# 17LiQi/MultimodalSignal

Hardware: AMD Instinct MI355X
Metric: train windows/sec (higher is better)
Workload: dtype f32; 1 GPU; CnnGruAttentionModel full train step (fwd+CE+bwd+Adam, dropout 0.5, BN batch stats), B=8192 windows/GPU x (6 ch, 3840 samples = 60 s @ 64 Hz), random-init weights; BASELINE.json configs[4] shape, the per-step work of configs[1]; batch_per_gpu=8192, channels=6, samples=3840, classes=2, parallelism=replica x1

## Files before the change

multimodalsignal_amd/csrc/frontend.hip:

```cpp
#include "msig_dev.h"

template <int CT, bool EO_ONLY = false>
__global__ __launch_bounds__(256) void gate_kernel(const float* __restrict__ x, const float* __restrict__ W1,
                                                   const float* __restrict__ W2, float* __restrict__ mean_out,
                                                   float* __restrict__ pre_out, float* __restrict__ s_out,
                                                   float* __restrict__ eo_out, int C, int T, int Cr, const FoldCtx fc) {
  FOLD_BEGIN; FS(x); FS(W1); FS(W2); FS(mean_out); FS(pre_out); FS(s_out); FS(eo_out);
  __shared__ float red[4][MSIG_MAX_C];
  __shared__ float red_eo[4][2 * MSIG_MAX_C];
  __shared__ float mean_s[MSIG_MAX_C];
  __shared__ float hid_s[MSIG_MAX_C / 4];
  const int b = blockIdx.x, tid = threadIdx.x, lane = tid & 63, w = tid >> 6;
  const float* xb = x + (size_t)b * C * T;
  if (CT > 0 && (T & 3) == 0) {
    constexpr int CN = CT > 0 ? CT : 1;
    float acc[CN], ev[CN], od[CN];
#pragma unroll
    for (int c = 0; c < CN; ++c) acc[c] = ev[c] = od[c] = 0.f;
    const int T4 = T / 4;
    constexpr int U = CN <= 4 ? 4 : 2;
    for (int i0 = tid; i0 < T4; i0 += 256 * U) {
      float4 q[U][CN];
#pragma unroll
      for (int u = 0; u < U; ++u) {
        const int i = i0 + 256 * u < T4 ? i0 + 256 * u : i0;
#pragma unroll
        for (int c = 0; c < CN; ++c) q[u][c] = ((const float4*)xb)[(size_t)c * T4 + i];
      }
#pragma unroll
      for (int u = 0; u < U; ++u)
        if (i0 + 256 * u < T4) {
#pragma unroll
          for (int c = 0; c < CN; ++c) {
            if (!EO_ONLY) acc[c] += (q[u][c].x + q[u][c].y) + (q[u][c].z + q[u][c].w);
            ev[c] += q[u][c].x + q[u][c].z; od[c] += q[u][c].y + q[u][c].w;
          }
        }
    }
#pragma unroll
    for (int c = 0; c < CN; ++c) {
      if (!EO_ONLY) {
        const float a = wave_sum(acc[c]);
        if (lane == 0) red[w][c] = a;
      }
      if (eo_out) {
        const float e = wave_sum(ev[c]), o = wave_sum(od[c]);
        if (lane == 0) { red_eo[w][2 * c] = e; red_eo[w][2 * c + 1] = o; }
      }
    }
  } else
  for (int c = 0; c < C; ++c) {
    const float* xc = xb + (size_t)c * T;
    float acc = 0.f, ev = 0.f, od = 0.f;
// ... 502 lines not shown
  __shared__ float red[256 * 8];
  const int c4 = threadIdx.x % C4;
  float s1[4] = {0.f, 0.f, 0.f, 0.f}, s2[4] = {0.f, 0.f, 0.f, 0.f};
  float mean[4], invstd[4];
#pragma unroll
  for (int e = 0; e < 4; ++e) { mean[e] = stat[c4 * 4 + e]; invstd[e] = stat[CH + c4 * 4 + e]; }
  const int64_t total = (int64_t)B * L * C4;
  for (int64_t i = (int64_t)blockIdx.x * 256 + threadIdx.x; i < total; i += (int64_t)gridDim.x * 256) {
    const int64_t bt = i / C4;
    const int t = (int)(bt % L), b = (int)(bt / L);
    RoutedRaw r = routed_load<CH>(dp_a, code, b, t, P, c4);
    if (dp_b) {
      const RoutedRaw r2 = routed_load<CH>(dp_b, code, b, t, P, c4);
      r.g0.x += r2.g0.x; r.g0.y += r2.g0.y; r.g0.z += r2.g0.z; r.g0.w += r2.g0.w;
      r.g1.x += r2.g1.x; r.g1.y += r2.g1.y; r.g1.z += r2.g1.z; r.g1.w += r2.g1.w;
    }
    const float4 d = routed_dz(r, t, P);
    const float4 yq = *(const float4*)(y + ((size_t)b * L + t) * CH + c4 * 4);
    *(float4*)(dz + ((size_t)b * L + t) * CH + c4 * 4) = d;
    const float dv[4] = {d.x, d.y, d.z, d.w}, yv[4] = {yq.x, yq.y, yq.z, yq.w};
#pragma unroll
    for (int e = 0; e < 4; ++e) { s1[e] += dv[e]; s2[e] += dv[e] * (yv[e] - mean[e]) * invstd[e]; }
  }
#pragma unroll
  for (int e = 0; e < 4; ++e) { red[threadIdx.x * 8 + e] = s1[e]; red[threadIdx.x * 8 + 4 + e] = s2[e]; }
  __syncthreads();
  if (threadIdx.x < 2 * CH) {
    const int which = threadIdx.x / CH, ch = threadIdx.x % CH, cc4 = ch / 4, e = ch % 4;
    float acc = 0.f;
    for (int t = cc4; t < 256; t += C4) acc += red[t * 8 + which * 4 + e];
    part[(size_t)blockIdx.x * 2 * CH + threadIdx.x] = acc;
  }
}

__global__ __launch_bounds__(FIN_THREADS) void bn_bwd_finalize_kernel(const float* __restrict__ part, int nrows, int CH, double count,
                                                              float* __restrict__ cstat, float* __restrict__ dgamma,
                                                              float* __restrict__ dbeta, int batch_stats, const FoldCtx fc) {
  FOLD_BEGIN; FS(part); FS(cstat); FS(dgamma); FS(dbeta);
  __shared__ double red[FIN_THREADS];
  const int tid = threadIdx.x, ncol = 2 * CH;
  fin_colsums(part, nrows, ncol, red);
  if (tid < ncol) {
    const double s = red[tid];
    if (tid < CH) dbeta[tid] = (float)s; else dgamma[tid - CH] = (float)s;
    cstat[tid] = batch_stats ? (float)(s / count) : 0.f;
  }
}

#define D2_UCH 128
#define D2_ROWS (D2_UCH + 2)
#define D2_PS 36
#define W2_PROWS (2 * D2_UCH + 3)

__global__ __launch_bounds__(256) void conv2_bwd_kernel(const float* __restrict__ dz2, const float* __restrict__ y2,
                                                        const float* __restrict__ stat, const float* __restrict__ cstat,
                                                        const float* __restrict__ w2, const float* __restrict__ p1,
                                                        float* __restrict__ dp1, float* __restrict__ part, int B, int P1, int L2,
                                                        const FoldCtx fc) {
  FOLD_BEGIN; FS(dz2); FS(y2); FS(stat); FS(cstat); FS(w2); FS(p1); FS(dp1); FS(part);
  __shared__ __attribute__((aligned(16))) float ds_[D2_ROWS * D2_PS];
  __shared__ __attribute__((aligned(16))) float ps[W2_PROWS * C2_PS];
  const int tid = threadIdx.x, lane = tid & 63, w = tid >> 6, li = lane & 15, lq = lane >> 4;
  float Ae[24], Ao[16];
#pragma unroll
  for (int m = 0; m < 24; ++m) Ae[m] = w2[((lq * 8 + (m & 7)) * 16 + li) * 5 + 2 * (m >> 3)];
#pragma unroll
  for (int m = 0; m < 16; ++m) Ao[m] = w2[((lq * 8 + (m & 7)) * 16 + li) * 5 + 1 + 2 * (m >> 3)];
  f32x4 acc[2][5];
#pragma unroll
  for (int ob = 0; ob < 2; ++ob)
#pragma unroll
    for (int kk = 0; kk < 5; ++kk) acc[ob][kk] = (f32x4){0.f, 0.f, 0.f, 0.f};
  const int nchunk = (L2 + D2_UCH - 1) / D2_UCH;
  const int nitems = B * nchunk;
  float bn_mean[4], bn_inv[4], bn_sc[4], bn_c1[4], bn_c2[4];
#pragma unroll
  for (int e = 0; e < 4; ++e) {
    const int ch = (tid & 7) * 4 + e;
    bn_mean[e] = stat[ch]; bn_inv[e] = stat[32 + ch]; bn_sc[e] = stat[64 + ch]; bn_c1[e] = cstat[ch]; bn_c2[e] = cstat[32 + ch];
  }
  constexpr int ND4 = (D2_ROWS * 8 + 255) / 256, NP4 = (W2_PROWS * 4 + 255) / 256;
  float4 dr[ND4], yr[ND4], qr[NP4];
  auto prefetch = [&](int item) {
    const int b = item / nchunk, t0 = (item - b * nchunk) * D2_UCH, base = 2 * t0 - 2;
#pragma unroll
    for (int j = 0; j < ND4; ++j) {
      const int i = tid + 256 * j, row = i >> 3, c4 = i & 7, t = t0 - 1 + row;
      const int tc = t < 0 ? 0 : (t > L2 - 1 ? L2 - 1 : t);
      dr[j] = *(const float4*)(dz2 + ((size_t)b * L2 + tc) * 32 + c4 * 4);
      yr[j] = *(const float4*)(y2 + ((size_t)b * L2 + tc) * 32 + c4 * 4);
    }
#pragma unroll
    for (int j = 0; j < NP4; ++j) {
      const int i = tid + 256 * j, row = i >> 2, c4 = i & 3, src = base + row;
      const int sc = src < 0 ? 0 : (src > P1 - 1 ? P1 - 1 : src);
      qr[j] = *(const float4*)(p1 + ((size_t)b * P1 + sc) * 16 + c4 * 4);
    }
  };
  if ((int)blockIdx.x < nitems) prefetch(blockIdx.x);
  for (int item = blockIdx.x; item < nitems; item += gridDim.x) {
    const int b = item / nchunk, t0 = (item - b * nchunk) * D2_UCH;
    __syncthreads();
#pragma unroll
    for (int j = 0; j < ND4; ++j) {
      const int i = tid + 256 * j, row = i >> 3, c4 = i & 7, t = t0 - 1 + row;
      if (i < D2_ROWS * 8) {
        const float4 dzv = dr[j];
        float4 q;
        q.x = bn_sc[0] * (dzv.x - bn_c1[0] - (yr[j].x - bn_mean[0]) * bn_inv[0] * bn_c2[0]);
        q.y = bn_sc[1] * (dzv.y - bn_c1[1] - (yr[j].y - bn_mean[1]) * bn_inv[1] * bn_c2[1]);
        q.z = bn_sc[2] * (dzv.z - bn_c1[2] - (yr[j].z - bn_mean[2]) * bn_inv[2] * bn_c2[2]);
        q.w = bn_sc[3] * (dzv.w - bn_c1[3] - (yr[j].w - bn_mean[3]) * bn_inv[3] * bn_c2[3]);
        if (t < 0 || t >= L2) q = make_float4(0.f, 0.f, 0.f, 0.f);
        *(float4*)&ds_[row * D2_PS + c4 * 4] = q;
      }
    }
    const int base = 2 * t0 - 2;
#pragma unroll
    for (int j = 0; j < NP4; ++j) {
      const int i = tid + 256 * j, row = i >> 2, c4 = i & 3, src = base + row;
      if (i < W2_PROWS * 4) {
        float4 q = qr[j];
        if (src < 0 || src >= P1) q = make_float4(0.f, 0.f, 0.f, 0.f);
        *(float4*)&ps[row * C2_PS + c4 * 4] = q;
      }
    }
    __syncthreads();
    if (item + (int)gridDim.x < nitems) prefetch(item + gridDim.x);
#pragma unroll
    for (int ubi = 0; ubi < 2; ++ubi) {
      const int ul = (w * 2 + ubi) * 16 + li;
      f32x4 ae0 = {0.f, 0.f, 0.f, 0.f}, ae1 = {0.f, 0.f, 0.f, 0.f}, ao0 = {0.f, 0.f, 0.f, 0.f}, ao1 = {0.f, 0.f, 0.f, 0.f};
#pragma unroll
      for (int ti = 0; ti < 3; ++ti) {
        const float* rowp = &ds_[(ul + 2 - ti) * D2_PS + lq * 8];
        const float4 q0 = *(const float4*)rowp, q1 = *(const float4*)(rowp + 4);
        const float qv[8] = {q0.x, q0.y, q0.z, q0.w, q1.x, q1.y, q1.z, q1.w};
#pragma unroll
        for (int mm = 0; mm < 8; ++mm) {
          if (mm & 1) ae1 = mfma16(Ae[ti * 8 + mm], qv[mm], ae1); else ae0 = mfma16(Ae[ti * 8 + mm], qv[mm], ae0);
          if (ti < 2) { if (mm & 1) ao1 = mfma16(Ao[ti * 8 + mm], qv[mm], ao1); else ao0 = mfma16(Ao[ti * 8 + mm], qv[mm], ao0); }
        }
      }
      const int u = t0 + ul;
      if (2 * u < P1)
        *(float4*)(dp1 + ((size_t)b * P1 + 2 * u) * 16 + lq * 4) = make_float4(ae0[0] + ae1[0], ae0[1] + ae1[1], ae0[2] + ae1[2], ae0[3] + ae1[3]);
      if (2 * u + 1 < P1)
        *(float4*)(dp1 + ((size_t)b * P1 + 2 * u + 1) * 16 + lq * 4) = make_float4(ao0[0] + ao1[0], ao0[1] + ao1[1], ao0[2] + ao1[2], ao0[3] + ao1[3]);
    }
#pragma unroll 2
    for (int m = 0; m < D2_UCH / 16; ++m) {
      const int tl = w * 32 + 4 * m + lq;
      const float a0 = ds_[(tl + 1) * D2_PS + li], a1 = ds_[(tl + 1) * D2_PS + 16 + li];
#pragma unroll
      for (int kk = 0; kk < 5; ++kk) {
        const float bv = ps[(2 * tl + kk) * C2_PS + li];
        acc[0][kk] = mfma16(a0, bv, acc[0][kk]);
        acc[1][kk] = mfma16(a1, bv, acc[1][kk]);
      }
    }
  }
  __syncthreads();
  float* red = ds_;
  for (int ww = 0; ww < 4; ++ww) {
    if (w == ww) {
#pragma unroll
      for (int ob = 0; ob < 2; ++ob)
#pragma unroll
        for (int kk = 0; kk < 5; ++kk)
#pragma unroll
          for (int e = 0; e < 4; ++e) {
            const int o = ob * 16 + lq * 4 + e, c = li;
            const int idx = (o * 16 + c) * 5 + kk;
            red[idx] = (ww == 0 ? 0.f : red[idx]) + acc[ob][kk][e];
          }
    }
    __syncthreads();
  }
  for (int i = tid; i < 2560; i += 256) part[(size_t)blockIdx.x * 2560 + i] = red[i];
}

struct QuadRaw { float4 g[3], y[4]; unsigned c[3]; };
__device__ __forceinline__ void quad_load(QuadRaw& r, const float* __restrict__ dp1, const uint8_t* __restrict__ code1,
                                          const float* __restrict__ y1, int b, int tq, int L1, int P1, int sc4) {
  const int tqc = tq < L1 - 4 ? tq : L1 - 4;
  const int ph = tqc >> 1, ph2 = ph + 2 < P1 ? ph + 2 : P1 - 1;
  const float* dpb = dp1 + (size_t)b * P1 * 16;
  const uint8_t* cb = code1 + (size_t)b * P1 * 4;
  const float* yb = y1 + (size_t)b * L1 * 16;
  const unsigned o = (unsigned)(ph * 16 + sc4 * 4), oc = (unsigned)(ph * 4 + sc4), oy = (unsigned)(tqc * 16 + sc4 * 4);
  r.g[0] = *(const float4*)(dpb + o); r.g[1] = *(const float4*)(dpb + o + 16); r.g[2] = *(const float4*)(dpb + (unsigned)(ph2 * 16 + sc4 * 4));
  r.c[0] = cb[oc]; r.c[1] = cb[oc + 4]; r.c[2] = cb[(unsigned)(ph2 * 4 + sc4)];
#pragma unroll
  for (int j = 0; j < 4; ++j) r.y[j] = *(const float4*)(yb + oy + 16 * j);
}
__device__ __forceinline__ void quad_dz_xhat(const QuadRaw& r, int tq, int L1, int P1, const float* bn_mean, const float* bn_inv,
                                             float4 dz[4], float4 xh[4]) {
  const bool inside = tq < L1, has2 = (tq >> 1) + 2 < P1;
  const float g0[4] = {r.g[0].x, r.g[0].y, r.g[0].z, r.g[0].w}, g1[4] = {r.g[1].x, r.g[1].y, r.g[1].z, r.g[1].w},
              g2[4] = {r.g[2].x, r.g[2].y, r.g[2].z, r.g[2].w};
  float d[4][4];
#pragma unroll
  for (int e = 0; e < 4; ++e) {
    const unsigned c0 = (r.c[0] >> (2 * e)) & 3u, c1 = (r.c[1] >> (2 * e)) & 3u, c2 = has2 ? (r.c[2] >> (2 * e)) & 3u : 3u;
    d[0][e] = c0 == 1u ? g0[e] : 0.f;
    d[1][e] = (c0 == 2u ? g0[e] : 0.f) + (c1 == 0u ? g1[e] : 0.f);
    d[2][e] = c1 == 1u ? g1[e] : 0.f;
    d[3][e] = (c1 == 2u ? g1[e] : 0.f) + (c2 == 0u ? g2[e] : 0.f);
  }
#pragma unroll
  for (int j = 0; j < 4; ++j) {
    float4 dq = make_float4(d[j][0], d[j][1], d[j][2], d[j][3]), h;
    h.x = (r.y[j].x - bn_mean[0]) * bn_inv[0];
    h.y = (r.y[j].y - bn_mean[1]) * bn_inv[1];
    h.z = (r.y[j].z - bn_mean[2]) * bn_inv[2];
    h.w = (r.y[j].w - bn_mean[3]) * bn_inv[3];
    if (!inside) { dq = make_float4(0.f, 0.f, 0.f, 0.f); h = dq; }
    dz[j] = dq; xh[j] = h;
  }
}

#define G1_TCH 256
#ifndef CONV1_BWD_PIPE
#define CONV1_BWD_PIPE 1
#endif
#define CONV1_BWD_WGS (CONV1_BWD_PIPE ? 2 : 4)
#define G1_MAXNB 7
#define G1_XS (C1_XW + 4)
#define G1_QS 80
__device__ __forceinline__ int g1_row(int r) { return (r >> 2) * G1_QS + (r & 3) * 16; }

__host__ __device__ inline int conv1_bwd_cps(int B, int nchunk) { return B >= 256 ? nchunk : (nchunk + 7) / 8; }
// ... 89 lines not shown
          h.y = (yv.y - bn_mean[1]) * bn_inv[1];
          h.z = (yv.z - bn_mean[2]) * bn_inv[2];
          h.w = (yv.w - bn_mean[3]) * bn_inv[3];
          if (t >= L1) { dq = make_float4(0.f, 0.f, 0.f, 0.f); h = dq; }
          *(float4*)&dzs[g1_row(row) + c4 * 4] = dq;
          *(float4*)&xhs[g1_row(row) + c4 * 4] = h;
        }
      }
      __syncthreads();
      if (pipe) {
        if (ch + 1 < ch_hi) prefetch(b, ch + 1);
        else if (item + (int)gridDim.x < nitems) { const int ni = item + gridDim.x; prefetch(ni / SEG, (ni % SEG) * CPS); }
      }
#pragma unroll
      for (int m = 0; m < G1_TCH / 16; ++m) {
        const float a1 = dzs[aoff + G1_QS * m], a2 = xhs[aoff + G1_QS * m];
        s1 += a1; s2 = fmaf(a1, a2, s2);
#pragma unroll
        for (int nb = 0; nb < NBC; ++nb)
          if (CT > 0 || nb < NB) {
            const float bv = xs[coff[nb] + 8 * m];
            acc1[nb] = mfma16(a1, bv, acc1[nb]);
            acc2[nb] = mfma16(a2, bv, acc2[nb]);
          }
      }
    }
    __syncthreads();
#pragma unroll
    for (int nb = 0; nb < NBC; ++nb)
      if (CT > 0 || nb < NB) {
#pragma unroll
        for (int e = 0; e < 4; ++e) {
          red[((w * 2 + 0) * 16 + lq * 4 + e) * NB16 + nb * 16 + li] = acc1[nb][e];
          red[((w * 2 + 1) * 16 + lq * 4 + e) * NB16 + nb * 16 + li] = acc2[nb][e];
        }
      }
    __syncthreads();
    {
      float* gw = g1w + (size_t)item * 32 * NB16;
      for (int i = tid; i < 32 * NB16; i += 256)
        gw[i] = (red[i] + red[32 * NB16 + i]) + (red[64 * NB16 + i] + red[96 * NB16 + i]);
    }
  }
  __syncthreads();
  red[(w * 4 + lq) * 32 + li] = s1;
  red[(w * 4 + lq) * 32 + 16 + li] = s2;
  __syncthreads();
  if (tid < 32) {
    float a = 0.f;
    for (int q = 0; q < 16; ++q) a += red[q * 32 + tid];
    bpart[(size_t)blockIdx.x * 32 + tid] = a;
  }
}

template <bool GATED = true>
__global__ __launch_bounds__(256) void conv1_bwd_fin_kernel(const float* __restrict__ g1w, const float* __restrict__ stat,
                                                            const float* __restrict__ cstat, const float* __restrict__ w1,
                                                            const float* __restrict__ gate_s, const float* __restrict__ eo,
                                                            const float* __restrict__ x, float* __restrict__ part,
                                                            float* __restrict__ ds_out, int B, int C, int T, int L1, int SEG, const FoldCtx fc) {
  FOLD_BEGIN; FS(g1w); FS(stat); FS(cstat); FS(w1); FS(gate_s); FS(eo); FS(x); FS(part); FS(ds_out);
  __shared__ float prod[16 * G1_MAXNB * 16];
  __shared__ float pc[16 * MSIG_MAX_C];
  __shared__ float ss[MSIG_MAX_C];
  __shared__ float sxs[G1_MAXNB * 16];
  const int K = C * 7, NB = (K + 15) / 16, NB16 = NB * 16, tid = threadIdx.x;
  float dwacc[G1_MAXNB], wv[G1_MAXNB], sc[G1_MAXNB], k1[G1_MAXNB], k2[G1_MAXNB];
  int col_[G1_MAXNB];
#pragma unroll
  for (int j = 0; j < G1_MAXNB; ++j) {
    const int idx = tid + 256 * j, o = (idx / NB16) & 15, col = idx % NB16;
    const bool ok = j < NB && col < K;
    dwacc[j] = 0.f;
    col_[j] = ok ? col : -1;
    wv[j] = ok ? w1[o * K + col] : 0.f;
    sc[j] = stat[32 + o]; k1[j] = cstat[o]; k2[j] = cstat[16 + o];
  }
  for (int b = blockIdx.x; b < B; b += gridDim.x) {
    const float* gw = g1w + (size_t)b * SEG * 32 * NB16;
    if (GATED && tid < C) ss[tid] = gate_s[(size_t)b * C + tid];
    if (tid >= 64 && tid < 64 + K) {
      const int col = tid - 64, c = col / 7, d = col - 7 * c - 3, par = d & 1;
      const float* xc = x + ((size_t)b * C + c) * T;
      float a = eo[((size_t)b * C + c) * 2 + par];
      for (int i = par; i < d; i += 2) a -= xc[i];
      for (int i = 2 * (L1 - 1) + d + 2; i < T; i += 2) if (i >= 0) a -= xc[i];
      sxs[col] = a;
    }
    __syncthreads();
#pragma unroll
    for (int j = 0; j < G1_MAXNB; ++j)
      if (j < NB) {
        const int idx = tid + 256 * j;
        float g = 0.f;
        if (col_[j] >= 0) {
          float gdz = gw[idx], gxh = gw[16 * NB16 + idx];
          for (int s0 = 1; s0 < SEG; s0 += 8) {
            float a8[8], b8[8];
#pragma unroll
            for (int u = 0; u < 8; ++u) {
              const int sg = s0 + u < SEG ? s0 + u : SEG - 1;
              a8[u] = gw[(size_t)sg * 32 * NB16 + idx]; b8[u] = gw[(size_t)sg * 32 * NB16 + 16 * NB16 + idx];
            }
#pragma unroll
            for (int u = 0; u < 8; ++u)
              if (s0 + u < SEG) { gdz += a8[u]; gxh += b8[u]; }
// ... 187 lines not shown
    switch (d.C) {
      case 1: GATE(1); break; case 2: GATE(2); break; case 3: GATE(3); break; case 4: GATE(4); break;
      case 5: GATE(5); break; case 6: GATE(6); break; case 7: GATE(7); break; case 8: GATE(8); break;
      default: GATE(0); break;
    }
#undef GATE
    MSIG_LAUNCH_CHECK();
  }
  const int tr = b->training;
  const bool keep = msig_keeps(b);
  {
    const int nchunk = (d.L1 + C1_CHUNK - 1) / C1_CHUNK;
    const int grid = clampi((int64_t)d.B * nchunk, MSIG_PERSIST_WG);
    const int KM = (d.C * 7 + 3) / 4;
    size_t smem = (size_t)(2 * d.C * C1_XP + 4 * KM * 16) * sizeof(float);
    if (smem < 4 * 32 * sizeof(float)) smem = 4 * 32 * sizeof(float);
    {
      MSIG_K("conv1_fwd", st);
#define C1F(CT, G) conv1_fwd_kernel<CT, G><<<dim3(grid, 1, fc.n), 256, smem, st>>>(b->x, P + po[MSIG_P_CONV1_W], gs, w.p<float>(MSIG_WS_Y1), \
                                                             w.p<float>(MSIG_WS_BN1_PART), d.B, d.C, d.T, d.L1, tr, fc)
#define C1F_ALL(G) switch (d.C) { \
        case 1: C1F(1, G); break; case 2: C1F(2, G); break; case 3: C1F(3, G); break; case 4: C1F(4, G); break; \
        case 5: C1F(5, G); break; case 6: C1F(6, G); break; case 7: C1F(7, G); break; case 8: C1F(8, G); break; \
        default: C1F(0, G); break; }
      if (gated) { C1F_ALL(true) } else { C1F_ALL(false) }
#undef C1F_ALL
#undef C1F
    }
    MSIG_LAUNCH_CHECK();
    { MSIG_K("bn_finalize", st); bn_finalize_kernel<<<dim3(1, 1, fc.n), FIN_THREADS, 0, st>>>(w.p<float>(MSIG_WS_BN1_PART), grid, 16, (double)d.B * d.L1, P + po[MSIG_P_BN1_G],
                                          P + po[MSIG_P_BN1_B], b->bn_state, b->bn_state + 16, b->bn_count, b->bn_momentum,
                                          b->bn_eps, tr, w.p<float>(MSIG_WS_BN1_STAT), fc); }
    MSIG_LAUNCH_CHECK();
  }
  {
    const int nchunk = (d.L2 + C2_CHUNK - 1) / C2_CHUNK;
    const int grid = clampi((int64_t)d.B * nchunk, MSIG_PERSIST_WG);
    { MSIG_K("pool1_conv2_fwd", st); pool1_conv2_fwd_kernel<<<dim3(grid, 1, fc.n), 256, 0, st>>>(w.p<float>(MSIG_WS_Y1), w.p<float>(MSIG_WS_BN1_STAT), w.p<float>(MSIG_WS_P1),
                                            keep ? w.p<uint8_t>(MSIG_WS_POOLC1) : nullptr, P + po[MSIG_P_CONV2_W], w.p<float>(MSIG_WS_Y2),
                                            w.p<float>(MSIG_WS_BN2_PART), d.B, d.L1, d.P1, d.L2, tr, fc); }
    MSIG_LAUNCH_CHECK();
    { MSIG_K("bn_finalize", st); bn_finalize_kernel<<<dim3(1, 1, fc.n), FIN_THREADS, 0, st>>>(w.p<float>(MSIG_WS_BN2_PART), grid, 32, (double)d.B * d.L2, P + po[MSIG_P_BN2_G],
                                          P + po[MSIG_P_BN2_B], b->bn_state + 32, b->bn_state + 64, b->bn_count + 1,
                                          b->bn_momentum, b->bn_eps, tr, w.p<float>(MSIG_WS_BN2_STAT), fc); }
    MSIG_LAUNCH_CHECK();
    const int64_t n = (int64_t)d.B * d.TP * 8;
    { MSIG_K("bn_relu_pool_32", st); bn_relu_pool_kernel<32><<<dim3(clampi((n + 255) / 256, 8192), 1, fc.n), 256, 0, st>>>(w.p<float>(MSIG_WS_Y2), w.p<float>(MSIG_WS_BN2_STAT),
                                                                          w.p<float>(MSIG_WS_P2), keep ? w.p<uint8_t>(MSIG_WS_POOLC2) : nullptr, d.B, d.L2, d.TP, fc); }
    MSIG_LAUNCH_CHECK();
  }
  return 0;
}

int launch_frontend_bwd(const msig_batch* b, const StageDims& d, const WsPtrs& w, const int64_t* po, ColsumPlan& plan, const FoldCtx& fc, hipStream_t st,
                        bool gated) {
  const float* P = b->params;
  float* G = b->grads;
  const PartOffsets pof = part_offsets(d);
  float* part2 = w.p<float>(MSIG_WS_GRAD_PART) + pof.conv2;
  float* part1 = w.p<float>(MSIG_WS_GRAD_PART) + pof.conv1;
  float* bpart = w.p<float>(MSIG_WS_BNB_PART);
  float* cstat = w.p<float>(MSIG_WS_BNB_STAT);
  {
    const float* dxa = w.p<float>(MSIG_WS_DX0);
    const float* dxb = dxa + (size_t)d.B * d.TP * 32;
    const int grid = clampi(((int64_t)d.B * d.L2 * 8 + 255) / 256, MSIG_PERSIST_WG);
    { MSIG_K("pool_bn_bwd_pass1_32", st); pool_bn_bwd_pass1<32><<<dim3(grid, 1, fc.n), 256, 0, st>>>(dxa, dxb, w.p<uint8_t>(MSIG_WS_POOLC2), w.p<float>(MSIG_WS_Y2),
                                                w.p<float>(MSIG_WS_BN2_STAT), w.p<float>(MSIG_WS_DY2), bpart, d.B, d.L2, d.TP, fc); }
    MSIG_LAUNCH_CHECK();
    { MSIG_K("bn_bwd_finalize", st); bn_bwd_finalize_kernel<<<dim3(1, 1, fc.n), FIN_THREADS, 0, st>>>(bpart, grid, 32, (double)d.B * d.L2, cstat, G + po[MSIG_P_BN2_G], G + po[MSIG_P_BN2_B], b->training, fc); }
    MSIG_LAUNCH_CHECK();
  }
  {
    const int gdw = clampi((int64_t)d.B * ((d.L2 + D2_UCH - 1) / D2_UCH), MSIG_CONV_DW_WG);
    { MSIG_K("conv2_bwd", st); conv2_bwd_kernel<<<dim3(gdw, 1, fc.n), 256, 0, st>>>(w.p<float>(MSIG_WS_DY2), w.p<float>(MSIG_WS_Y2), w.p<float>(MSIG_WS_BN2_STAT), cstat,
                                                                          P + po[MSIG_P_CONV2_W], w.p<float>(MSIG_WS_P1), w.p<float>(MSIG_WS_DP1), part2,
                                                                          d.B, d.P1, d.L2, fc); }
    MSIG_LAUNCH_CHECK();
    if (!plan.add(part2, gdw, 2560, 0, 2560, G + po[MSIG_P_CONV2_W])) return MSIG_E_SHAPE;
  }
  {
    const int K = d.C * 7, NB = (K + 15) / 16;
    const int nchunk1 = (d.L1 + G1_TCH - 1) / G1_TCH, seg = conv1_bwd_segs(d.B, nchunk1);
    const int grid = clampi((int64_t)d.B * seg, MSIG_CONV_DW_WG), grid_fin = clampi(d.B, MSIG_CONV_DW_WG);
    size_t smem = (size_t)(d.C * G1_XS + 2 * (G1_TCH / 4) * G1_QS) * sizeof(float);
    if (smem < (size_t)128 * NB * 16 * sizeof(float)) smem = (size_t)128 * NB * 16 * sizeof(float);
    float* g1w = w.p<float>(MSIG_WS_G1W);
    {
      MSIG_K("conv1_bwd", st);
#define C1B(CT) conv1_bwd_kernel<CT><<<dim3(grid, 1, fc.n), 256, smem, st>>>(w.p<float>(MSIG_WS_DP1), w.p<uint8_t>(MSIG_WS_POOLC1), w.p<float>(MSIG_WS_Y1), w.p<float>(MSIG_WS_BN1_STAT), b->x, \
                                                             g1w, bpart, d.B, d.C, d.T, d.L1, d.P1, fc)
      switch (d.C) {
        case 1: C1B(1); break; case 2: C1B(2); break; case 3: C1B(3); break; case 4: C1B(4); break;
        case 5: C1B(5); break; case 6: C1B(6); break; case 7: C1B(7); break; case 8: C1B(8); break;
        default: C1B(0); break;
      }
#undef C1B
    }
    MSIG_LAUNCH_CHECK();
    { MSIG_K("bn_bwd_finalize", st); bn_bwd_finalize_kernel<<<dim3(1, 1, fc.n), FIN_THREADS, 0, st>>>(bpart, grid, 16, (double)d.B * d.L1, cstat, G + po[MSIG_P_BN1_G], G + po[MSIG_P_BN1_B], b->training, fc); }
    MSIG_LAUNCH_CHECK();
    {
      MSIG_K("conv1_bwd_fin", st);
      if (gated)
        conv1_bwd_fin_kernel<true><<<dim3(grid_fin, 1, fc.n), 256, 0, st>>>(g1w, w.p<float>(MSIG_WS_BN1_STAT), cstat, P + po[MSIG_P_CONV1_W], w.p<float>(MSIG_WS_GATE_S),
                                                                            w.p<float>(MSIG_WS_GATE_EO), b->x, part1, w.p<float>(MSIG_WS_DS), d.B, d.C, d.T, d.L1, seg, fc);
      else
        conv1_bwd_fin_kernel<false><<<dim3(grid_fin, 1, fc.n), 256, 0, st>>>(g1w, w.p<float>(MSIG_WS_BN1_STAT), cstat, P + po[MSIG_P_CONV1_W], nullptr,
                                                                             w.p<float>(MSIG_WS_GATE_EO), b->x, part1, nullptr, d.B, d.C, d.T, d.L1, seg, fc);
    }
    MSIG_LAUNCH_CHECK();
    if (!plan.add(part1, grid_fin, 16 * K, 0, 16 * K, G + po[MSIG_P_CONV1_W])) return MSIG_E_SHAPE;
    if (b->dx) {
      const int nchunk_dx = (d.L1 + DX_UCH - 1) / DX_UCH;
      {
        MSIG_K("conv1_bwd_dx", st);
        if (gated)
          conv1_bwd_dx_kernel<true><<<dim3(d.B * nchunk_dx, 1, fc.n), 256, 0, st>>>(w.p<float>(MSIG_WS_DP1), w.p<uint8_t>(MSIG_WS_POOLC1),
              w.p<float>(MSIG_WS_Y1), w.p<float>(MSIG_WS_BN1_STAT), cstat, P + po[MSIG_P_CONV1_W], w.p<float>(MSIG_WS_GATE_S), w.p<float>(MSIG_WS_GATE_PRE),
              P + po[MSIG_P_GATE_W1], P + po[MSIG_P_GATE_W2], w.p<float>(MSIG_WS_DS), b->dx, d.C, d.Cr, d.T, d.L1, d.P1, fc);
        else
          conv1_bwd_dx_kernel<false><<<dim3(d.B * nchunk_dx, 1, fc.n), 256, 0, st>>>(w.p<float>(MSIG_WS_DP1), w.p<uint8_t>(MSIG_WS_POOLC1),
              w.p<float>(MSIG_WS_Y1), w.p<float>(MSIG_WS_BN1_STAT), cstat, P + po[MSIG_P_CONV1_W], nullptr, nullptr, nullptr, nullptr, nullptr,
              b->dx, d.C, 0, d.T, d.L1, d.P1, fc);
      }
      MSIG_LAUNCH_CHECK();
    }
    if (gated && d.Cr > 0) {
      { MSIG_K("gate_bwd", st); gate_bwd_kernel<<<dim3(2 * d.C * d.Cr, 1, fc.n), 256, 0, st>>>(w.p<float>(MSIG_WS_DS), w.p<float>(MSIG_WS_GATE_S), w.p<float>(MSIG_WS_GATE_PRE),
                                                        w.p<float>(MSIG_WS_GATE_MEAN), P + po[MSIG_P_GATE_W2], G + po[MSIG_P_GATE_W1],
                                                        G + po[MSIG_P_GATE_W2], d.B, d.C, d.Cr, fc); }
      MSIG_LAUNCH_CHECK();
    }
  }
  return 0;
}
```

Before: 1.055 million windows/s.

## Add warp-specialized double-buffered loader/compute variants of conv2 and conv1 backward

Adds 512-thread warp-specialized kernels for the conv2 and conv1 backward passes. In each, 256 loader threads prefetch global data, apply the BN backward transform and stage it into double-buffered dynamic LDS, while 256 compute threads run the MFMA contractions, with register lookahead and sched barriers around the LDS reads. The dp1 store is also reshuffled with xor-8 shuffles so each lane writes a contiguous row. The aim is to overlap global loads with MFMA work in these persistent kernels. The cost is doubled threads and LDS per block, which lowers occupancy, plus a mutex-guarded LDS opt-in.

```diff
diff --git a/multimodalsignal_amd/csrc/frontend.hip b/multimodalsignal_amd/csrc/frontend.hip
--- a/multimodalsignal_amd/csrc/frontend.hip
+++ b/multimodalsignal_amd/csrc/frontend.hip
@@ -1,4 +1,5 @@
 #include "msig_dev.h"
+#include <mutex>
 
 template <int CT, bool EO_ONLY = false>
 __global__ __launch_bounds__(256) void gate_kernel(const float* __restrict__ x, const float* __restrict__ W1,
@@ -607,6 +608,97 @@
 #define D2_PS 36
 #define W2_PROWS (2 * D2_UCH + 3)
 
+template <bool AHEAD>
+__device__ __forceinline__ void conv2_bwd_contract(const float* ds_, const float* ps, const float (&Ae)[24], const float (&Ao)[16],
+                                                   f32x4 (&acc)[2][5], float* __restrict__ dp1, int b, int t0, int P1, int w, int li, int lq) {
+  float4 q[2][3][2];
+  auto read_dx = [&](int ubi) {
+    const int ul = (w * 2 + ubi) * 16 + li;
+#pragma unroll
+    for (int ti = 0; ti < 3; ++ti) {
+      const float* rowp = &ds_[(ul + 2 - ti) * D2_PS + lq * 8];
+      q[ubi][ti][0] = *(const float4*)rowp; q[ubi][ti][1] = *(const float4*)(rowp + 4);
+    }
+  };
+  float da0[2], da1[2], dbv[2][5];
+  auto read_dw = [&](int m) {
+    const int tl = w * 32 + 4 * m + lq;
+    da0[m & 1] = ds_[(tl + 1) * D2_PS + li]; da1[m & 1] = ds_[(tl + 1) * D2_PS + 16 + li];
+#pragma unroll
+    for (int kk = 0; kk < 5; ++kk) dbv[m & 1][kk] = ps[(2 * tl + kk) * C2_PS + li];
+  };
+  if (AHEAD) read_dx(0);
+#pragma unroll
+  for (int ubi = 0; ubi < 2; ++ubi) {
+    const int ul = (w * 2 + ubi) * 16 + li;
+    if (AHEAD) {
+      if (ubi == 0) read_dx(1); else read_dw(0);
+      __builtin_amdgcn_sched_barrier(0);
+    } else {
+      read_dx(ubi);
+    }
+    f32x4 ae0 = {0.f, 0.f, 0.f, 0.f}, ae1 = {0.f, 0.f, 0.f, 0.f}, ao0 = {0.f, 0.f, 0.f, 0.f}, ao1 = {0.f, 0.f, 0.f, 0.f};
+#pragma unroll
+    for (int ti = 0; ti < 3; ++ti) {
+      const float4 q0 = q[ubi][ti][0], q1 = q[ubi][ti][1];
+      const float qv[8] = {q0.x, q0.y, q0.z, q0.w, q1.x, q1.y, q1.z, q1.w};
+#pragma unroll
+      for (int mm = 0; mm < 8; ++mm) {
+        if (mm & 1) ae1 = mfma16(Ae[ti * 8 + mm], qv[mm], ae1); else ae0 = mfma16(Ae[ti * 8 + mm], qv[mm], ae0);
+        if (ti < 2) { if (mm & 1) ao1 = mfma16(Ao[ti * 8 + mm], qv[mm], ao1); else ao0 = mfma16(Ao[ti * 8 + mm], qv[mm], ao0); }
+      }
+    }
+    if (AHEAD) __builtin_amdgcn_sched_barrier(0);
+    const float4 ev = make_float4(ae0[0] + ae1[0], ae0[1] + ae1[1], ae0[2] + ae1[2], ae0[3] + ae1[3]);
+    const float4 od = make_float4(ao0[0] + ao1[0], ao0[1] + ao1[1], ao0[2] + ao1[2], ao0[3] + ao1[3]);
+    const bool lo = li < 8;
+    const float rx = __shfl_xor(lo ? od.x : ev.x, 8), ry = __shfl_xor(lo ? od.y : ev.y, 8);
+    const float rz = __shfl_xor(lo ? od.z : ev.z, 8), rw = __shfl_xor(lo ? od.w : ev.w, 8);
+    const int u = t0 + ul;
+    const int r1 = lo ? 2 * u : 2 * (u - 8) + 1;
+    const int r2 = lo ? 2 * (u + 8) : 2 * u + 1;
+    if (r1 < P1) *(float4*)(dp1 + ((size_t)b * P1 + r1) * 16 + lq * 4) = make_float4(lo ? ev.x : rx, lo ? ev.y : ry, lo ? ev.z : rz, lo ? ev.w : rw);
+    if (r2 < P1) *(float4*)(dp1 + ((size_t)b * P1 + r2) * 16 + lq * 4) = make_float4(lo ? rx : od.x, lo ? ry : od.y, lo ? rz : od.z, lo ? rw : od.w);
+  }
+  if (AHEAD) {
+#pragma unroll
+    for (int m = 0; m < D2_UCH / 16; ++m) {
+      if (m + 1 < D2_UCH / 16) read_dw(m + 1);
+      __builtin_amdgcn_sched_barrier(0);
+#pragma unroll
+      for (int kk = 0; kk < 5; ++kk) {
+        acc[0][kk] = mfma16(da0[m & 1], dbv[m & 1][kk], acc[0][kk]);
+        acc[1][kk] = mfma16(da1[m & 1], dbv[m & 1][kk], acc[1][kk]);
+      }
+      __builtin_amdgcn_sched_barrier(0);
+    }
+  } else {
+#pragma unroll 2
+    for (int m = 0; m < D2_UCH / 16; ++m) {
+      const int tl = w * 32 + 4 * m + lq;
+      const float a0 = ds_[(tl + 1) * D2_PS + li], a1 = ds_[(tl + 1) * D2_PS + 16 + li];
+#pragma unroll
+      for (int kk = 0; kk < 5; ++kk) {
+        const float bv = ps[(2 * tl + kk) * C2_PS + li];
+        acc[0][kk] = mfma16(a0, bv, acc[0][kk]);
+        acc[1][kk] = mfma16(a1, bv, acc[1][kk]);
+      }
+    }
+  }
+}
+__device__ __forceinline__ void conv2_bwd_reduce(float* red, const f32x4 (&acc)[2][5], bool first, int li, int lq) {
+#pragma unroll
+  for (int ob = 0; ob < 2; ++ob)
+#pragma unroll
+    for (int kk = 0; kk < 5; ++kk)
+#pragma unroll
+      for (int e = 0; e < 4; ++e) {
+        const int o = ob * 16 + lq * 4 + e, c = li;
+        const int idx = (o * 16 + c) * 5 + kk;
+        red[idx] = (first ? 0.f : red[idx]) + acc[ob][kk][e];
+      }
+}
+
 __global__ __launch_bounds__(256) void conv2_bwd_kernel(const float* __restrict__ dz2, const float* __restrict__ y2,
                                                         const float* __restrict__ stat, const float* __restrict__ cstat,
                                                         const float* __restrict__ w2, const float* __restrict__ p1,
@@ -682,57 +774,131 @@
     }
     __syncthreads();
     if (item + (int)gridDim.x < nitems) prefetch(item + gridDim.x);
-#pragma unroll
-    for (int ubi = 0; ubi < 2; ++ubi) {
-      const int ul = (w * 2 + ubi) * 16 + li;
-      f32x4 ae0 = {0.f, 0.f, 0.f, 0.f}, ae1 = {0.f, 0.f, 0.f, 0.f}, ao0 = {0.f, 0.f, 0.f, 0.f}, ao1 = {0.f, 0.f, 0.f, 0.f};
-#pragma unroll
-      for (int ti = 0; ti < 3; ++ti) {
-        const float* rowp = &ds_[(ul + 2 - ti) * D2_PS + lq * 8];
-        const float4 q0 = *(const float4*)rowp, q1 = *(const float4*)(rowp + 4);
-        const float qv[8] = {q0.x, q0.y, q0.z, q0.w, q1.x, q1.y, q1.z, q1.w};
-#pragma unroll
-        for (int mm = 0; mm < 8; ++mm) {
-          if (mm & 1) ae1 = mfma16(Ae[ti * 8 + mm], qv[mm], ae1); else ae0 = mfma16(Ae[ti * 8 + mm], qv[mm], ae0);
-          if (ti < 2) { if (mm & 1) ao1 = mfma16(Ao[ti * 8 + mm], qv[mm], ao1); else ao0 = mfma16(Ao[ti * 8 + mm], qv[mm], ao0); }
-        }
-      }
-      const int u = t0 + ul;
-      if (2 * u < P1)
-        *(float4*)(dp1 + ((size_t)b * P1 + 2 * u) * 16 + lq * 4) = make_float4(ae0[0] + ae1[0], ae0[1] + ae1[1], ae0[2] + ae1[2], ae0[3] + ae1[3]);
-      if (2 * u + 1 < P1)
-        *(float4*)(dp1 + ((size_t)b * P1 + 2 * u + 1) * 16 + lq * 4) = make_float4(ao0[0] + ao1[0], ao0[1] + ao1[1], ao0[2] + ao1[2], ao0[3] + ao1[3]);
-    }
-#pragma unroll 2
-    for (int m = 0; m < D2_UCH / 16; ++m) {
-      const int tl = w * 32 + 4 * m + lq;
-      const float a0 = ds_[(tl + 1) * D2_PS + li], a1 = ds_[(tl + 1) * D2_PS + 16 + li];
-#pragma unroll
-      for (int kk = 0; kk < 5; ++kk) {
-        const float bv = ps[(2 * tl + kk) * C2_PS + li];
-        acc[0][kk] = mfma16(a0, bv, acc[0][kk]);
-        acc[1][kk] = mfma16(a1, bv, acc[1][kk]);
-      }
-    }
+    conv2_bwd_contract<false>(ds_, ps, Ae, Ao, acc, dp1, b, t0, P1, w, li, lq);
   }
   __syncthreads();
   float* red = ds_;
   for (int ww = 0; ww < 4; ++ww) {
-    if (w == ww) {
-#pragma unroll
-      for (int ob = 0; ob < 2; ++ob)
-#pragma unroll
-        for (int kk = 0; kk < 5; ++kk)
-#pragma unroll
-          for (int e = 0; e < 4; ++e) {
-            const int o = ob * 16 + lq * 4 + e, c = li;
-            const int idx = (o * 16 + c) * 5 + kk;
-            red[idx] = (ww == 0 ? 0.f : red[idx]) + acc[ob][kk][e];
-          }
-    }
+    if (w == ww) conv2_bwd_reduce(red, acc, ww == 0, li, lq);
     __syncthreads();
   }
   for (int i = tid; i < 2560; i += 256) part[(size_t)blockIdx.x * 2560 + i] = red[i];
+}
+
+#define D2_STAGE (D2_ROWS * D2_PS + W2_PROWS * C2_PS)
+#define D2_WS_SMEM (2 * D2_STAGE * sizeof(float))
+__global__ __launch_bounds__(512) void conv2_bwd_ws_kernel(const float* __restrict__ dz2, const float* __restrict__ y2,
+                                                           const float* __restrict__ stat, const float* __restrict__ cstat,
+                                                           const float* __restrict__ w2, const float* __restrict__ p1,
+                                                           float* __restrict__ dp1, float* __restrict__ part, int B, int P1, int L2,
+                                                           const FoldCtx fc) {
+  FOLD_BEGIN; FS(dz2); FS(y2); FS(stat); FS(cstat); FS(w2); FS(p1); FS(dp1); FS(part);
+  extern __shared__ __attribute__((aligned(16))) float smem[];
+  const int tid = threadIdx.x & 255, lane = tid & 63, w = tid >> 6, li = lane & 15, lq = lane >> 4;
+  const bool loader = threadIdx.x >= 256;
+  const int nchunk = (L2 + D2_UCH - 1) / D2_UCH;
+  const int nitems = B * nchunk, G = gridDim.x, it0 = blockIdx.x;
+  float* red = smem;
+  if (loader) {
+    float bn_mean[4], bn_inv[4], bn_sc[4], bn_c1[4], bn_c2[4];
+#pragma unroll
+    for (int e = 0; e < 4; ++e) {
+      const int ch = (tid & 7) * 4 + e;
+      bn_mean[e] = stat[ch]; bn_inv[e] = stat[32 + ch]; bn_sc[e] = stat[64 + ch]; bn_c1[e] = cstat[ch]; bn_c2[e] = cstat[32 + ch];
+    }
+    constexpr int ND4 = (D2_ROWS * 8 + 255) / 256, NP4 = (W2_PROWS * 4 + 255) / 256;
+    struct Raw { float4 dr[ND4], yr[ND4], qr[NP4]; };
+    Raw ra, rb;
+    auto prefetch = [&](Raw& r, int item) {
+      const int b = item / nchunk, t0 = (item - b * nchunk) * D2_UCH, base = 2 * t0 - 2;
+#pragma unroll
+      for (int j = 0; j < ND4; ++j) {
+        const int i = tid + 256 * j, row = i >> 3, c4 = i & 7, t = t0 - 1 + row;
+        const int tc = t < 0 ? 0 : (t > L2 - 1 ? L2 - 1 : t);
+        r.dr[j] = *(const float4*)(dz2 + ((size_t)b * L2 + tc) * 32 + c4 * 4);
+        r.yr[j] = *(const float4*)(y2 + ((size_t)b * L2 + tc) * 32 + c4 * 4);
+      }
+#pragma unroll
+      for (int j = 0; j < NP4; ++j) {
+        const int i = tid + 256 * j, row = i >> 2, c4 = i & 3, src = base + row;
+        const int sc = src < 0 ? 0 : (src > P1 - 1 ? P1 - 1 : src);
+        r.qr[j] = *(const float4*)(p1 + ((size_t)b * P1 + sc) * 16 + c4 * 4);
+      }
+    };
+    auto stage = [&](const Raw& r, int item, float* ds_, float* ps) {
+      const int b = item / nchunk, t0 = (item - b * nchunk) * D2_UCH;
+#pragma unroll
+      for (int j = 0; j < ND4; ++j) {
+        const int i = tid + 256 * j, row = i >> 3, c4 = i & 7, t = t0 - 1 + row;
+        if (i < D2_ROWS * 8) {
+          const float4 dzv = r.dr[j];
+          float4 q;
+          q.x = bn_sc[0] * (dzv.x - bn_c1[0] - (r.yr[j].x - bn_mean[0]) * bn_inv[0] * bn_c2[0]);
+          q.y = bn_sc[1] * (dzv.y - bn_c1[1] - (r.yr[j].y - bn_mean[1]) * bn_inv[1] * bn_c2[1]);
+          q.z = bn_sc[2] * (dzv.z - bn_c1[2] - (r.yr[j].z - bn_mean[2]) * bn_inv[2] * bn_c2[2]);
+          q.w = bn_sc[3] * (dzv.w - bn_c1[3] - (r.yr[j].w - bn_mean[3]) * bn_inv[3] * bn_c2[3]);
+          if (t < 0 || t >= L2) q = make_float4(0.f, 0.f, 0.f, 0.f);
+          *(float4*)&ds_[row * D2_PS + c4 * 4] = q;
+        }
+      }
+      const int base = 2 * t0 - 2;
+#pragma unroll
+      for (int j = 0; j < NP4; ++j) {
+        const int i = tid + 256 * j, row = i >> 2, c4 = i & 3, src = base + row;
+        if (i < W2_PROWS * 4) {
+          float4 q = r.qr[j];
+          if (src < 0 || src >= P1) q = make_float4(0.f, 0.f, 0.f, 0.f);
+          *(float4*)&ps[row * C2_PS + c4 * 4] = q;
+        }
+      }
+    };
+    float* s0 = smem;
+    float* s1 = smem + D2_STAGE;
+    if (it0 < nitems) prefetch(ra, it0);
+    if (it0 + G < nitems) prefetch(rb, it0 + G);
+    if (it0 < nitems) {
+      stage(ra, it0, s0, s0 + D2_ROWS * D2_PS);
+      if (it0 + 2 * G < nitems) prefetch(ra, it0 + 2 * G);
+      lds_barrier();
+    }
+    for (int item = it0; item < nitems; item += 2 * G) {
+      if (item + G < nitems) {
+        stage(rb, item + G, s1, s1 + D2_ROWS * D2_PS);
+        if (item + 3 * G < nitems) prefetch(rb, item + 3 * G);
+        lds_barrier();
+      }
+      if (item + 2 * G < nitems) {
+        stage(ra, item + 2 * G, s0, s0 + D2_ROWS * D2_PS);
+        if (item + 4 * G < nitems) prefetch(ra, item + 4 * G);
+        lds_barrier();
+      }
+    }
+    for (int k = 0; k < 5; ++k) lds_barrier();
+  } else {
+    float Ae[24], Ao[16];
+#pragma unroll
+    for (int m = 0; m < 24; ++m) Ae[m] = w2[((lq * 8 + (m & 7)) * 16 + li) * 5 + 2 * (m >> 3)];
+#pragma unroll
+    for (int m = 0; m < 16; ++m) Ao[m] = w2[((lq * 8 + (m & 7)) * 16 + li) * 5 + 1 + 2 * (m >> 3)];
+    f32x4 acc[2][5];
+#pragma unroll
+    for (int ob = 0; ob < 2; ++ob)
+#pragma unroll
+      for (int kk = 0; kk < 5; ++kk) acc[ob][kk] = (f32x4){0.f, 0.f, 0.f, 0.f};
+    int s = 0;
+    for (int item = it0; item < nitems; item += G, s ^= 1) {
+      const int b = item / nchunk, t0 = (item - b * nchunk) * D2_UCH;
+      const float* ds_ = smem + s * D2_STAGE;
+      lds_barrier();
+      conv2_bwd_contract<true>(ds_, ds_ + D2_ROWS * D2_PS, Ae, Ao, acc, dp1, b, t0, P1, w, li, lq);
+    }
+    lds_barrier();
+    for (int ww = 0; ww < 4; ++ww) {
+      if (w == ww) conv2_bwd_reduce(red, acc, ww == 0, li, lq);
+      lds_barrier();
+    }
+  }
+  for (int i = threadIdx.x; i < 2560; i += 512) part[(size_t)blockIdx.x * 2560 + i] = red[i];
 }
 
 struct QuadRaw { float4 g[3], y[4]; unsigned c[3]; };
@@ -928,6 +1094,173 @@
     bpart[(size_t)blockIdx.x * 32 + tid] = a;
   }
 }
+
+template <int CT>
+__global__ __launch_bounds__(512) void conv1_bwd_ws_kernel(const float* __restrict__ dp1, const uint8_t* __restrict__ code1,
+                                                           const float* __restrict__ y1, const float* __restrict__ stat,
+                                                           const float* __restrict__ x, float* __restrict__ g1w,
+                                                           float* __restrict__ bpart, int B, int T, int L1, int P1, const FoldCtx fc) {
+  FOLD_BEGIN; FS(dp1); FS(code1); FS(y1); FS(stat); FS(x); FS(g1w); FS(bpart);
+  extern __shared__ __attribute__((aligned(16))) float smem[];
+  constexpr int C = CT, K = C * 7, NB = (K + 15) / 16, NB16 = NB * 16;
+  constexpr int STAGE = C * G1_XS + 2 * (G1_TCH / 4) * G1_QS;
+  float* red = smem + 2 * STAGE;
+  const int tid = threadIdx.x & 255, lane = tid & 63, w = tid >> 6, li = lane & 15, lq = lane >> 4;
+  const bool loader = threadIdx.x >= 256;
+  const int nchunk = (L1 + G1_TCH - 1) / G1_TCH;
+  const int CPS = conv1_bwd_cps(B, nchunk), SEG = conv1_bwd_segs(B, nchunk), nitems = B * SEG, G = gridDim.x;
+  struct Cur { int item, b, ch, hi; };
+  auto cur_set = [&](Cur& c, int item) {
+    c.item = item;
+    if (item < nitems) {
+      c.b = item / SEG;
+      c.ch = (item - c.b * SEG) * CPS;
+      c.hi = c.ch + CPS < nchunk ? c.ch + CPS : nchunk;
+    }
+  };
+  auto cur_adv = [&](Cur& c) { if (++c.ch >= c.hi) cur_set(c, c.item + G); };
+  float s1 = 0.f, s2 = 0.f;
+  bool pending = false;
+  int pend_item = 0;
+  auto flush = [&]() {
+    float* gw = g1w + (size_t)pend_item * 32 * NB16;
+    for (int i = tid; i < 32 * NB16; i += 256)
+      gw[i] = (red[i] + red[32 * NB16 + i]) + (red[64 * NB16 + i] + red[96 * NB16 + i]);
+  };
+  if (loader) {
+    float bn_mean[4], bn_inv[4];
+#pragma unroll
+    for (int e = 0; e < 4; ++e) {
+      const int ch = (tid & 3) * 4 + e;
+      bn_mean[e] = stat[ch]; bn_inv[e] = stat[16 + ch];
+    }
+    constexpr int NX4 = (CT * (C1_XW / 4) + 255) / 256;
+    const int sq = tid >> 2, sc4 = tid & 3;
+    struct Raw { float4 xr[NX4]; QuadRaw q; };
+    Raw ra, rb;
+    auto prefetch = [&](Raw& r, const Cur& c) {
+      const int t0 = c.ch * G1_TCH, g_base = 2 * t0 - 4;
+      const float* xb = x + (size_t)c.b * C * T;
+#pragma unroll
+      for (int j = 0; j < NX4; ++j) {
+        const int i = tid + 256 * j, ic = i < C * (C1_XW / 4) ? i : 0;
+        const int cc = ic / (C1_XW / 4), i4 = ic - cc * (C1_XW / 4), g0 = g_base + 4 * i4;
+        const int gc = g0 < 0 ? 0 : (g0 > T - 4 ? T - 4 : g0);
+        r.xr[j] = *(const float4*)(xb + (unsigned)(cc * T + gc));
+      }
+      quad_load(r.q, dp1, code1, y1, c.b, t0 + 4 * sq, L1, P1, sc4);
+    };
+    auto stage = [&](const Raw& r, int ch, float* xs) {
+      float* dzs = xs + C * G1_XS;
+      float* xhs = dzs + (G1_TCH / 4) * G1_QS;
+      const int t0 = ch * G1_TCH, g_base = 2 * t0 - 4;
+#pragma unroll
+      for (int j = 0; j < NX4; ++j) {
+        const int i = tid + 256 * j;
+        if (i < C * (C1_XW / 4)) {
+          const int cc = i / (C1_XW / 4), i4 = i - cc * (C1_XW / 4), g0 = g_base + 4 * i4;
+          float4 q = r.xr[j];
+          if (g0 < 0 || g0 > T - 4) q = make_float4(0.f, 0.f, 0.f, 0.f);
+          *(float4*)&xs[cc * G1_XS + 4 * i4] = q;
+        }
+      }
+      float4 dq[4], h[4];
+      quad_dz_xhat(r.q, t0 + 4 * sq, L1, P1, bn_mean, bn_inv, dq, h);
+#pragma unroll
+      for (int j = 0; j < 4; ++j) {
+        *(float4*)&dzs[sq * G1_QS + j * 16 + sc4 * 4] = dq[j];
+        *(float4*)&xhs[sq * G1_QS + j * 16 + sc4 * 4] = h[j];
+      }
+    };
+    Cur pf, sg;
+    cur_set(pf, blockIdx.x);
+    cur_set(sg, blockIdx.x);
+    if (pf.item < nitems) { prefetch(ra, pf); cur_adv(pf); }
+    if (pf.item < nitems) { prefetch(rb, pf); cur_adv(pf); }
+    if (sg.item < nitems) {
+      stage(ra, sg.ch, smem); cur_adv(sg);
+      if (pf.item < nitems) { prefetch(ra, pf); cur_adv(pf); }
+      lds_barrier();
+    }
+    while (sg.item < nitems) {
+      stage(rb, sg.ch, smem + STAGE); cur_adv(sg);
+      if (pf.item < nitems) { prefetch(rb, pf); cur_adv(pf); }
+      lds_barrier();
+      if (sg.item >= nitems) break;
+      stage(ra, sg.ch, smem); cur_adv(sg);
+      if (pf.item < nitems) { prefetch(ra, pf); cur_adv(pf); }
+      lds_barrier();
+    }
+  } else {
+    int coff[NB];
+#pragma unroll
+    for (int nb = 0; nb < NB; ++nb) {
+      const int col = nb * 16 + li, cc = col < K ? col : K - 1, c = cc / 7, kk = cc - 7 * c;
+      coff[nb] = c * G1_XS + kk + 1 + 2 * (w * 64 + lq);
+    }
+    const int aoff = (w * 16) * G1_QS + lq * 16 + li;
+    f32x4 acc1[NB], acc2[NB];
+#pragma unroll
+    for (int nb = 0; nb < NB; ++nb) { acc1[nb] = (f32x4){0.f, 0.f, 0.f, 0.f}; acc2[nb] = (f32x4){0.f, 0.f, 0.f, 0.f}; }
+    Cur c;
+    cur_set(c, blockIdx.x);
+    int s = 0;
+    while (c.item < nitems) {
+      lds_barrier();
+      if (pending) { flush(); pending = false; }
+      const float* xs = smem + s * STAGE;
+      const float* dzs = xs + C * G1_XS;
+      const float* xhs = dzs + (G1_TCH / 4) * G1_QS;
+      float a1[2], a2[2], bv[2][NB];
+      auto read_k = [&](int m) {
+        a1[m & 1] = dzs[aoff + G1_QS * m]; a2[m & 1] = xhs[aoff + G1_QS * m];
+#pragma unroll
+        for (int nb = 0; nb < NB; ++nb) bv[m & 1][nb] = xs[coff[nb] + 8 * m];
+      };
+      read_k(0);
+#pragma unroll
+      for (int m = 0; m < G1_TCH / 16; ++m) {
+        if (m + 1 < G1_TCH / 16) read_k(m + 1);
+        __builtin_amdgcn_sched_barrier(0);
+        s1 += a1[m & 1]; s2 = fmaf(a1[m & 1], a2[m & 1], s2);
+#pragma unroll
+        for (int nb = 0; nb < NB; ++nb) {
+          acc1[nb] = mfma16(a1[m & 1], bv[m & 1][nb], acc1[nb]);
+          acc2[nb] = mfma16(a2[m & 1], bv[m & 1][nb], acc2[nb]);
+        }
+        __builtin_amdgcn_sched_barrier(0);
+      }
+      s ^= 1;
+      if (c.ch + 1 >= c.hi) {
+#pragma unroll
+        for (int nb = 0; nb < NB; ++nb) {
+#pragma unroll
+          for (int e = 0; e < 4; ++e) {
+            red[((w * 2 + 0) * 16 + lq * 4 + e) * NB16 + nb * 16 + li] = acc1[nb][e];
+            red[((w * 2 + 1) * 16 + lq * 4 + e) * NB16 + nb * 16 + li] = acc2[nb][e];
+          }
+          acc1[nb] = (f32x4){0.f, 0.f, 0.f, 0.f}; acc2[nb] = (f32x4){0.f, 0.f, 0.f, 0.f};
+        }
+        pending = true; pend_item = c.item;
+      }
+      cur_adv(c);
+    }
+  }
+  __syncthreads();
+  if (!loader && pending) flush();
+  __syncthreads();
+  if (!loader) {
+    red[(w * 4 + lq) * 32 + li] = s1;
+    red[(w * 4 + lq) * 32 + 16 + li] = s2;
+  }
+  __syncthreads();
+  if (threadIdx.x < 32) {
+    float a = 0.f;
+    for (int q = 0; q < 16; ++q) a += red[q * 32 + threadIdx.x];
+    bpart[(size_t)blockIdx.x * 32 + threadIdx.x] = a;
+  }
+}
+#define G1_WS_SMEM(C) ((size_t)(2 * ((C) * G1_XS + 2 * (G1_TCH / 4) * G1_QS) + 128 * (((C) * 7 + 15) / 16 * 16)) * sizeof(float))
 
 template <bool GATED = true>
 __global__ __launch_bounds__(256) void conv1_bwd_fin_kernel(const float* __restrict__ g1w, const float* __restrict__ stat,
@@ -1221,6 +1554,21 @@
   return 0;
 }
 
+static int frontend_lds_optin() {
+  static std::mutex mu;
+  static bool done[64] = {};
+  int dev = 0;
+  hipError_t e = hipGetDevice(&dev);
+  if (e != hipSuccess) return (int)e;
+  if (dev < 0 || dev >= 64) return MSIG_E_SHAPE;
+  std::lock_guard<std::mutex> lk(mu);
+  if (done[dev]) return 0;
+  if ((e = hipFuncSetAttribute((const void*)conv2_bwd_ws_kernel, hipFuncAttributeMaxDynamicSharedMemorySize, (int)D2_WS_SMEM)) != hipSuccess) return (int)e;
+  if ((e = hipFuncSetAttribute((const void*)conv1_bwd_ws_kernel<6>, hipFuncAttributeMaxDynamicSharedMemorySize, (int)G1_WS_SMEM(6))) != hipSuccess) return (int)e;
+  done[dev] = true;
+  return 0;
+}
+
 int launch_frontend_bwd(const msig_batch* b, const StageDims& d, const WsPtrs& w, const int64_t* po, ColsumPlan& plan, const FoldCtx& fc, hipStream_t st,
                         bool gated) {
   const float* P = b->params;
@@ -1241,10 +1589,21 @@
     MSIG_LAUNCH_CHECK();
   }
   {
-    const int gdw = clampi((int64_t)d.B * ((d.L2 + D2_UCH - 1) / D2_UCH), MSIG_CONV_DW_WG);
-    { MSIG_K("conv2_bwd", st); conv2_bwd_kernel<<<dim3(gdw, 1, fc.n), 256, 0, st>>>(w.p<float>(MSIG_WS_DY2), w.p<float>(MSIG_WS_Y2), w.p<float>(MSIG_WS_BN2_STAT), cstat,
-                                                                          P + po[MSIG_P_CONV2_W], w.p<float>(MSIG_WS_P1), w.p<float>(MSIG_WS_DP1), part2,
-                                                                          d.B, d.P1, d.L2, fc); }
+    const int64_t items2 = (int64_t)d.B * ((d.L2 + D2_UCH - 1) / D2_UCH);
+    const int gdw = clampi(items2, MSIG_CONV_DW_WG);
+    const bool ws2 = items2 > gdw;
+    if (ws2) { const int rc = frontend_lds_optin(); if (rc) return rc; }
+    {
+      MSIG_K("conv2_bwd", st);
+      if (ws2)
+        conv2_bwd_ws_kernel<<<dim3(gdw, 1, fc.n), 512, D2_WS_SMEM, st>>>(w.p<float>(MSIG_WS_DY2), w.p<float>(MSIG_WS_Y2), w.p<float>(MSIG_WS_BN2_STAT), cstat,
+                                                                        P + po[MSIG_P_CONV2_W], w.p<float>(MSIG_WS_P1), w.p<float>(MSIG_WS_DP1), part2,
+                                                                        d.B, d.P1, d.L2, fc);
+      else
+        conv2_bwd_kernel<<<dim3(gdw, 1, fc.n), 256, 0, st>>>(w.p<float>(MSIG_WS_DY2), w.p<float>(MSIG_WS_Y2), w.p<float>(MSIG_WS_BN2_STAT), cstat,
+                                                             P + po[MSIG_P_CONV2_W], w.p<float>(MSIG_WS_P1), w.p<float>(MSIG_WS_DP1), part2,
+                                                             d.B, d.P1, d.L2, fc);
+    }
     MSIG_LAUNCH_CHECK();
     if (!plan.add(part2, gdw, 2560, 0, 2560, G + po[MSIG_P_CONV2_W])) return MSIG_E_SHAPE;
   }
@@ -1255,7 +1614,13 @@
     size_t smem = (size_t)(d.C * G1_XS + 2 * (G1_TCH / 4) * G1_QS) * sizeof(float);
     if (smem < (size_t)128 * NB * 16 * sizeof(float)) smem = (size_t)128 * NB * 16 * sizeof(float);
     float* g1w = w.p<float>(MSIG_WS_G1W);
-    {
+    const bool ws1 = d.C == 6 && CONV1_BWD_PIPE && (d.T & 7) == 0 && 2 * d.P1 == d.L1 && d.L1 >= 8 && conv1_bwd_cps(d.B, nchunk1) >= 2;
+    if (ws1) { const int rc = frontend_lds_optin(); if (rc) return rc; }
+    if (ws1) {
+      MSIG_K("conv1_bwd", st);
+      conv1_bwd_ws_kernel<6><<<dim3(grid, 1, fc.n), 512, G1_WS_SMEM(6), st>>>(w.p<float>(MSIG_WS_DP1), w.p<uint8_t>(MSIG_WS_POOLC1), w.p<float>(MSIG_WS_Y1), w.p<float>(MSIG_WS_BN1_STAT), b->x,
+                                                                             g1w, bpart, d.B, d.T, d.L1, d.P1, fc);
+    } else {
       MSIG_K("conv1_bwd", st);
 #define C1B(CT) conv1_bwd_kernel<CT><<<dim3(grid, 1, fc.n), 256, smem, st>>>(w.p<float>(MSIG_WS_DP1), w.p<uint8_t>(MSIG_WS_POOLC1), w.p<float>(MSIG_WS_Y1), w.p<float>(MSIG_WS_BN1_STAT), b->x, \
                                                              g1w, bpart, d.B, d.C, d.T, d.L1, d.P1, fc)
```

Measured after the change: 1.036 million windows/s. 0.982x the previous value.
